# danieleschmidt/connectome-gnn-suite

Measured on AMD Instinct MI355X. Metric: training graphs/sec, 3-layer GCN, batch=4096x360-ROI connectomes, higher is better.
Workload: dtype f32; 1 GPU; cfg4-headline-gcn-4096x360-h64; model=gcn, rois=360, ws_k=14, edges_per_graph=5040, hidden=64, layers=3, node_order=dataset, graphs_per_gpu=4096, global_batch=4096, optimizer=Adam lr1e-3 wd1e-4 (optim.Adam), impl=fused, launch=eager, bn=per-rank, rccl_ranks=0, parallelism=graph-sharded dp1

## Files before the change

connectome_gnn_amd/csrc/common.h:

```cpp
#pragma once
#include <hip/hip_runtime.h>
#include <stdint.h>
#include "../../include/cgnn.h"

#define CGNN_WAVE 64

#define CGNN_CHECK_LAUNCH()                                   \
  do {                                                        \
    if (hipGetLastError() != hipSuccess) return CGNN_ELAUNCH; \
  } while (0)

#define CGNN_NEED_BYTES(ptr, have, need)                                   \
  do {                                                                     \
    if ((ptr) && (int64_t)(have) < (int64_t)(need)) return CGNN_EINVAL;    \
  } while (0)

static inline hipStream_t cgnn_stream(void* s) { return reinterpret_cast<hipStream_t>(s); }

#define CGNN_MAX_DEVICES 64
static inline int cgnn_device_ordinal() {
  int d = 0;
  if (hipGetDevice(&d) != hipSuccess || d < 0 || d >= CGNN_MAX_DEVICES) return 0;
  return d;
}

static inline int64_t cgnn_align_up(int64_t x, int64_t a) { return (x + a - 1) / a * a; }

__device__ __forceinline__ int cgnn_uniform(int v) { return __builtin_amdgcn_readfirstlane(v); }

__device__ __forceinline__ float cgnn_wave_sum(float v) {
#pragma unroll
  for (int o = 32; o > 0; o >>= 1) v += __shfl_xor(v, o, 64);
  return v;
}
__device__ __forceinline__ double cgnn_wave_sum(double v) {
#pragma unroll
  for (int o = 32; o > 0; o >>= 1) v += __shfl_xor(v, o, 64);
  return v;
}

__device__ __forceinline__ double block_sum256(double v, double* sh) {
  v = cgnn_wave_sum(v);
  if ((threadIdx.x & 63) == 0) sh[threadIdx.x >> 6] = v;
  __syncthreads();
  const double t = sh[0] + sh[1] + sh[2] + sh[3];
  __syncthreads();
  return t;
}

typedef float cgnn_f32x4 __attribute__((ext_vector_type(4)));
typedef uint32_t cgnn_u32x4 __attribute__((ext_vector_type(4)));
typedef uint32_t cgnn_u32x2 __attribute__((ext_vector_type(2)));
__device__ __forceinline__ float4 ldnt4(const float* p) {
  const cgnn_f32x4 v = __builtin_nontemporal_load(reinterpret_cast<const cgnn_f32x4*>(p));
  return make_float4(v[0], v[1], v[2], v[3]);
}
__device__ __forceinline__ void stnt4(float* p, const float4& v) {
  __builtin_nontemporal_store(cgnn_f32x4{v.x, v.y, v.z, v.w}, reinterpret_cast<cgnn_f32x4*>(p));
}
__device__ __forceinline__ float ldnt(const float* p) { return __builtin_nontemporal_load(p); }
__device__ __forceinline__ uint4 ldnt(const uint4* p) {
  const cgnn_u32x4 v = __builtin_nontemporal_load(reinterpret_cast<const cgnn_u32x4*>(p));
  return make_uint4(v[0], v[1], v[2], v[3]);
}
__device__ __forceinline__ uint2 ldnt(const uint2* p) {
  const cgnn_u32x2 v = __builtin_nontemporal_load(reinterpret_cast<const cgnn_u32x2*>(p));
  return make_uint2(v[0], v[1]);
}
```

connectome_gnn_amd/csrc/fused_gcn.hip:

```cpp
#include "common.h"
#include "agg_block.h"
#include "split_bf16.h"
#include "bn_coef.h"
#include "bn_tail.h"
#include "drop_ew.h"
#include "l0src.h"

#define PF_LD ld4
#define PF_ST st4
#define BW_LD ldnt4
#define BW_ST stnt4

#ifdef CGNN_STAMPS
__device__ unsigned long long g_stamps[1024 * 8 * 8];
#define CGNN_STAMP_DECL unsigned long long stamp_t_ = 0; (void)stamp_t_;
#define CGNN_STAMP_BEGIN() stamp_t_ = __builtin_amdgcn_s_memtime();
#define CGNN_STAMP(slot)                                                               \
  {                                                                                    \
    const unsigned long long now_ = __builtin_amdgcn_s_memtime();                      \
    if ((threadIdx.x & 63) == 0)                                                       \
      g_stamps[((size_t)blockIdx.x * 8 + (threadIdx.x >> 6)) * 8 + (slot)] += now_ - stamp_t_; \
    stamp_t_ = now_;                                                                   \
  }
#else
#define CGNN_STAMP_DECL
#define CGNN_STAMP_BEGIN()
#define CGNN_STAMP(slot)
#endif

namespace {

typedef float f32x4 __attribute__((ext_vector_type(4)));

constexpr int HID = CGNN_FUSED_HIDDEN;
constexpr int NWAVE = 8;
constexpr int NTHR = NWAVE * 64;
constexpr int SLD = 68;
constexpr int STG_FLOATS = 16 * SLD;

__device__ __forceinline__ float4 act4(const float4& y, const float4& a, const float4& b,
                                        uint32_t keep, float scale, float4& f) {
  float4 z, x;
  z.x = fmaf(a.x, y.x, b.x); z.y = fmaf(a.y, y.y, b.y);
  z.z = fmaf(a.z, y.z, b.z); z.w = fmaf(a.w, y.w, b.w);
  f.x = (z.x > 0.f && (keep & 1u)) ? scale : 0.f;
  f.y = (z.y > 0.f && (keep & 2u)) ? scale : 0.f;
  f.z = (z.z > 0.f && (keep & 4u)) ? scale : 0.f;
  f.w = (z.w > 0.f && (keep & 8u)) ? scale : 0.f;
  x.x = z.x * f.x; x.y = z.y * f.y; x.z = z.z * f.z; x.w = z.w * f.w;
  return x;
}

// ... 18 lines not shown
  __syncthreads();
  if (threadIdx.x < 128) {
    double t = 0.0;
#pragma unroll
    for (int w = 0; w < NW; ++w) t += red[w * 128 + threadIdx.x];
    slab_row[threadIdx.x] = t;
  }
  __syncthreads();
}

#define CGNN_FWD_G 4
#define CGNN_BWD_G 2
constexpr int FWD_G = CGNN_FWD_G;
constexpr int BWD_G = CGNN_BWD_G;

template <int MAXR, bool FIRST>
__global__ void __launch_bounds__(NTHR) k_gcn_fwd(
    cgnn_tiles t, const float* __restrict__ Xin, int F0, const float* __restrict__ bn_prev,
    DropCfg drop_in, int use_drop, uint8_t* __restrict__ mask_out, const float* __restrict__ W,
    const float* __restrict__ bias, float* __restrict__ Y, double* __restrict__ stat_slab) {
  const DropCfg drop = drop_resolve(drop_in);
  __shared__ __attribute__((aligned(16))) float tile[MAXR * HID];
  __shared__ __attribute__((aligned(16))) float stg_all[NWAVE * STG_FLOATS];
  __shared__ float disl[MAXR];
  const int lane = threadIdx.x & 63, wave = threadIdx.x >> 6, q = lane >> 4, j = lane & 15;
  float* stg = stg_all + wave * STG_FLOATS;
  const uint4* ent = static_cast<const uint4*>(t.ent_dst);

  __shared__ __attribute__((aligned(16))) float Wt[FIRST ? 4 : HID * HID];
  float wreg[4][4];
  if (FIRST) {
#pragma unroll
    for (int tj = 0; tj < 4; ++tj)
#pragma unroll
      for (int s = 0; s < 4; ++s) {
        const int k = 4 * s + q;
        wreg[tj][s] = k < F0 ? W[(4 * j + tj) * F0 + k] : 0.f;
      }
  } else {
    for (int i = threadIdx.x; i < HID * HID; i += NTHR) Wt[(i & 63) * HID + (i >> 6)] = W[i];
  }
  const float4 bias4 = ld4(bias + 4 * j);
  float4 pa = make_float4(0.f, 0.f, 0.f, 0.f), pb = pa;
  if (!FIRST) {
    pa = ld4(bn_prev + 4 * j);
    pb = ld4(bn_prev + HID + 4 * j);
  }
  double s1[4] = {0, 0, 0, 0}, s2[4] = {0, 0, 0, 0};
  CGNN_STAMP_DECL
  constexpr int PF = FIRST ? 1 : MAXR / 32;
  float4 pfy[PF];
  float pfd[PF];
  if (!FIRST && (int)blockIdx.x < t.num_tiles) {
    const int nb2 = t.tile_ptr[blockIdx.x], nn2 = t.tile_ptr[blockIdx.x + 1] - nb2;
#pragma unroll
    for (int u = 0; u < PF; ++u) {
      const int row = (threadIdx.x >> 4) + 32 * u;
      pfy[u] = make_float4(0.f, 0.f, 0.f, 0.f);
      pfd[u] = 0.f;
      if (row < nn2) {
        pfy[u] = ld4(Xin + (int64_t)(nb2 + row) * HID + 4 * j);
        pfd[u] = t.dis[nb2 + row];
      }
    }
  }

  for (int tid = blockIdx.x; tid < t.num_tiles; tid += gridDim.x) {
    CGNN_STAMP_BEGIN()
    const int base = t.tile_ptr[tid];
    const int n = t.tile_ptr[tid + 1] - base;
    const int nblk = (n + 15) >> 4;
    const int gb0 = t.tile_blk[tid];
    int boff[3] = {0, 0, 0}, bwid[3] = {0, 0, 0};
#pragma unroll
    for (int k = 0; k < 3; ++k) {
      const int bb = cgnn_uniform(wave) + NWAVE * k;
      if (bb < nblk) {
        boff[k] = t.blk_off_dst[gb0 + bb];
        bwid[k] = (t.blk_off_dst[gb0 + bb + 1] - boff[k]) >> 4;
      }
    }
    int off0 = boff[0], width = bwid[0], bk = 0;
    MetaRegs pre;
    if (wave < nblk) pre = meta_issue<true>(ent + (off0 >> 1), width, q, j);

    if (FIRST) {
      for (int r = threadIdx.x; r < nblk * 16; r += NTHR) disl[r] = r < n ? t.dis[base + r] : 0.f;
      for (int b = wave; b < nblk; b += NWAVE) {
        const int arow = 16 * b + j;
        f32x4 acc[4] = {{0, 0, 0, 0}, {0, 0, 0, 0}, {0, 0, 0, 0}, {0, 0, 0, 0}};
        float av[4], dv[4];
#pragma unroll
        for (int s = 0; s < 4; ++s) {
          const int k = 4 * s + q;
          av[s] = (arow < n && k < F0) ? Xin[(int64_t)(base + arow) * F0 + k] : 0.f;
          const int row = 16 * b + 4 * q + s;
          dv[s] = row < n ? t.dis[base + row] : 0.f;
        }
#pragma unroll
        for (int s = 0; s < 4; ++s)
          if (4 * s < F0) {
#pragma unroll
            for (int tj = 0; tj < 4; ++tj)
              acc[tj] = __builtin_amdgcn_mfma_f32_16x16x4f32(av[s], wreg[tj][s], acc[tj], 0, 0, 0);
          }
#pragma unroll
        for (int r = 0; r < 4; ++r)
          st4(tile + (16 * b + 4 * q + r) * HID + 4 * j,
              make_float4(acc[0][r] * dv[r], acc[1][r] * dv[r], acc[2][r] * dv[r], acc[3][r] * dv[r]));
      }
    } else {
#pragma unroll
      for (int u = 0; u < PF; ++u) {
        const int row = (threadIdx.x >> 4) + 32 * u;
        if (row < nblk * 16) {
          float4 x = make_float4(0.f, 0.f, 0.f, 0.f);
          if (row < n) {
            uint32_t keep = 0xFu;
            if (use_drop) {
              keep = drop_bits(drop, (uint32_t)(base + row) * 16u + (uint32_t)j);
              if (mask_out) mask_out[(int64_t)(base + row) * 16 + j] = (uint8_t)keep;
            }
            float4 f;
            x = scale4(act4(pfy[u], pa, pb, keep, drop.scale, f), pfd[u]);
          }
          st4(tile + row * HID + 4 * j, x);
          if (j == 0) disl[row] = pfd[u];
        }
      }
    }
    __syncthreads();
    if (!FIRST) {
      const int nxt = tid + gridDim.x;
      if (nxt < t.num_tiles) {
        const int nb2 = t.tile_ptr[nxt], nn2 = t.tile_ptr[nxt + 1] - nb2;
#pragma unroll
        for (int u = 0; u < PF; ++u) {
          const int row = (threadIdx.x >> 4) + 32 * u;
          pfy[u] = make_float4(0.f, 0.f, 0.f, 0.f);
          pfd[u] = 0.f;
          if (row < nn2) {
            pfy[u] = ld4(Xin + (int64_t)(nb2 + row) * HID + 4 * j);
            pfd[u] = t.dis[nb2 + row];
          }
        }
      }
    }
    CGNN_STAMP(1)

    for (int b = wave; b < nblk; b += NWAVE) {
      f32x4 acc[4] = {{0, 0, 0, 0}, {0, 0, 0, 0}, {0, 0, 0, 0}, {0, 0, 0, 0}};
      ++bk;
      const int off1 = bk == 1 ? boff[1] : boff[2], width1 = bk == 1 ? bwid[1] : bwid[2];
      CGNN_STAMP(2)
      float4 ag[4];
      agg_block<FWD_G, true>(tile, pre, ent + (off0 >> 1), width, q, j, ag);
      CGNN_STAMP(3)
      if (b + NWAVE < nblk) pre = meta_issue<true>(ent + (off1 >> 1), width1, q, j);
      off0 = off1; width = width1;
      if (FIRST) {
#pragma unroll
        for (int it = 0; it < 4; ++it) {
          const int row = 16 * b + 4 * q + it;
          if (row < n) {
            const float4 a = scale4(ag[it], disl[row]);
            const float4 y = make_float4(a.x + bias4.x, a.y + bias4.y, a.z + bias4.z, a.w + bias4.w);
            st4(Y + (int64_t)(base + row) * HID + 4 * j, y);
            s1[0] += y.x; s1[1] += y.y; s1[2] += y.z; s1[3] += y.w;
            s2[0] += (double)y.x * y.x; s2[1] += (double)y.y * y.y;
            s2[2] += (double)y.z * y.z; s2[3] += (double)y.w * y.w;
          }
        }
        CGNN_STAMP(4)
        continue;
      }
#pragma unroll
      for (int it = 0; it < 4; ++it)
        st4(stg + (4 * q + it) * SLD + 4 * j, scale4(ag[it], disl[16 * b + 4 * q + it]));
      __builtin_amdgcn_wave_barrier();
      float af[16];
#pragma unroll
      for (int u = 0; u < 4; ++u) {
        const float4 v = ld4(stg + j * SLD + 16 * q + 4 * u);
        af[4 * u + 0] = v.x; af[4 * u + 1] = v.y; af[4 * u + 2] = v.z; af[4 * u + 3] = v.w;
      }
      CGNN_STAMP(4)
#pragma unroll
      for (int s = 0; s < 16; ++s) {
// ... 45 lines not shown
}

constexpr int WSP_FRAGS = 3 * 2 * 4 * 64;
template <bool TRANSPOSED>
__device__ __forceinline__ void stage_split_weight(uint4* wsp, const float* __restrict__ W, int nthreads) {
  for (int idx = threadIdx.x; idx < 2 * 4 * 64; idx += nthreads) {
    const int ln = idx & 63, tj = (idx >> 6) & 3, ms = idx >> 8;
    const int qq = ln >> 4, jj = ln & 15;
    float v[8];
#pragma unroll
    for (int e = 0; e < 8; ++e) {
      const int k = 16 * (2 * ms + (e >> 2)) + 4 * qq + (e & 3), n = 4 * jj + tj;
      v[e] = TRANSPOSED ? W[k * HID + n] : W[n * HID + k];
    }
    const Split8 s = split8(make_float4(v[0], v[1], v[2], v[3]), make_float4(v[4], v[5], v[6], v[7]));
    wsp[((0 * 2 + ms) * 4 + tj) * 64 + ln] = s.h;
    wsp[((1 * 2 + ms) * 4 + tj) * 64 + ln] = s.m;
    wsp[((2 * 2 + ms) * 4 + tj) * 64 + ln] = s.l;
  }
}

constexpr int PF_NW = 12;
constexpr int PF_NTHR = PF_NW * 64;
#define CGNN_PF_G 2

template <int MAXR, bool FROM_P0>
__global__ void __launch_bounds__(PF_NTHR) k_gcn_fwd_pf(
    cgnn_tiles t, const float* __restrict__ Xin, cgnn_l0src l0, const float* __restrict__ bn_prev, DropCfg drop_in,
    int use_drop, uint8_t* __restrict__ mask_out, const float* __restrict__ W,
    const float* __restrict__ bias, float* __restrict__ Y, double* __restrict__ stat_slab, cgnn_bn_tail tail) {
  const DropCfg drop = drop_resolve(drop_in);
  __shared__ __attribute__((aligned(16))) float tile[MAXR * HID];
  __shared__ uint4 wsp[WSP_FRAGS];
  __shared__ __attribute__((aligned(16))) float bnab[2 * HID];
  __shared__ float disl[MAXR];
  const int lane = threadIdx.x & 63, wave = threadIdx.x >> 6, q = lane >> 4, j = lane & 15;
  const uint4* ent = static_cast<const uint4*>(t.ent_dst);
  constexpr int BPW = (MAXR / 16 + PF_NW - 1) / PF_NW;

  __shared__ __attribute__((aligned(16))) float b0l[FROM_P0 ? HID : 4];
  stage_split_weight<false>(wsp, W, PF_NTHR);
  for (int i = threadIdx.x; i < 2 * HID; i += PF_NTHR) bnab[i] = bn_prev[i];
  L0W w0;
  if (FROM_P0) {
    w0 = l0w_cols(l0, lane);
    for (int i = threadIdx.x; i < HID; i += PF_NTHR) b0l[i] = l0.b0[i];
  }
  const float4 bias4 = ld4(bias + 4 * j);
  double s1[4] = {0, 0, 0, 0}, s2[4] = {0, 0, 0, 0};

  constexpr int NPX = FROM_P0 ? 1 : 4;
  float4 px[BPW][NPX];
  float pd[BPW];
  auto request_block = [&](int tid, int u) {
    const int nb2 = t.tile_ptr[tid], nn2 = t.tile_ptr[tid + 1] - nb2;
    const int row = 16 * (wave + PF_NW * u) + j;
    pd[u] = 0.f;
#pragma unroll
    for (int c = 0; c < NPX; ++c) px[u][c] = make_float4(0.f, 0.f, 0.f, 0.f);
    if (row < nn2) {
      if (FROM_P0) {
        const float* src = l0.P0 + (int64_t)(nb2 + row) * L0_FP + q;
        px[u][0].x = src[0];
        px[u][0].y = src[4];
      } else {
        const float* src = Xin + (int64_t)(nb2 + row) * HID + 4 * q;
#pragma unroll
        for (int c = 0; c < NPX; ++c) px[u][c] = PF_LD(src + 16 * c);
      }
      pd[u] = t.dis[nb2 + row];
    }
  };
  auto request = [&](int tid) {
#pragma unroll
    for (int u = 0; u < BPW; ++u) request_block(tid, u);
  };
  if ((int)blockIdx.x < t.num_tiles) request(blockIdx.x);
  __syncthreads();

  for (int tid = blockIdx.x; tid < t.num_tiles; tid += gridDim.x) {
    const int base = t.tile_ptr[tid];
    const int n = t.tile_ptr[tid + 1] - base;
    const int nblk = (n + 15) >> 4;
    const int gb0 = t.tile_blk[tid];
    int boff[BPW], bwid[BPW];
#pragma unroll
    for (int k = 0; k < BPW; ++k) {
      boff[k] = bwid[k] = 0;
      const int bb = cgnn_uniform(wave) + PF_NW * k;
      if (bb < nblk) {
        boff[k] = t.blk_off_dst[gb0 + bb];
        bwid[k] = (t.blk_off_dst[gb0 + bb + 1] - boff[k]) >> 4;
      }
    }
    MetaRegs pre;
    if (wave < nblk) pre = meta_issue<true>(ent + (boff[0] >> 1), bwid[0], q, j);

    const int nxt = tid + gridDim.x;
#pragma unroll
    for (int u = 0; u < BPW; ++u) {
      const int b = wave + PF_NW * u;
      if (b >= nblk) break;
      const int row = 16 * b + j;
      const bool live = row < n;
      f32x4 acc[4] = {{0, 0, 0, 0}, {0, 0, 0, 0}, {0, 0, 0, 0}, {0, 0, 0, 0}};
#pragma unroll
      for (int ms = 0; ms < 2; ++ms) {
        float4 xc[2];
#pragma unroll
        for (int h2 = 0; h2 < 2; ++h2) {
          const int c = 2 * ms + h2;
          uint32_t keep = 0xFu;
          if (use_drop) {
            keep = drop_bits(drop, (uint32_t)(base + row) * 16u + (uint32_t)(4 * c + q));
            if (mask_out && live) mask_out[(int64_t)(base + row) * 16 + 4 * c + q] = (uint8_t)keep;
          }
          float4 f;
          float4 yraw = px[u][c < NPX ? c : 0];
          if (FROM_P0) {
            const float4 bq = ld4(b0l + 16 * c + 4 * q);
            const l0_f32x4 y0 = l0_mfma(w0.a[c], w0.b[c], px[u][0].x, px[u][0].y, l0_f32x4{bq.x, bq.y, bq.z, bq.w});
            yraw = make_float4(y0[0], y0[1], y0[2], y0[3]);
          }
          xc[h2] = scale4(act4(yraw, ld4(bnab + 16 * c + 4 * q), ld4(bnab + HID + 16 * c + 4 * q),
                               keep, drop.scale, f), pd[u]);
        }
        const Split8 a = split8(xc[0], xc[1]);
#pragma unroll
        for (int tj = 0; tj < 4; ++tj) {
          const uint4 bh = wsp[((0 * 2 + ms) * 4 + tj) * 64 + lane];
          const uint4 bm = wsp[((1 * 2 + ms) * 4 + tj) * 64 + lane];
          const uint4 bl = wsp[((2 * 2 + ms) * 4 + tj) * 64 + lane];
          acc[tj] = mfma_split(a, bh, bm, bl, acc[tj]);
        }
        __builtin_amdgcn_sched_barrier(0);
      }
#pragma unroll
      for (int r = 0; r < 4; ++r)
        st4(tile + (16 * b + 4 * q + r) * HID + 4 * j, make_float4(acc[0][r], acc[1][r], acc[2][r], acc[3][r]));
      if (q == 0) disl[row] = pd[u];
      if (nxt < t.num_tiles) request_block(nxt, u);
    }
    if (nxt < t.num_tiles) {
#pragma unroll
      for (int u = 0; u < BPW; ++u)
        if (wave + PF_NW * u >= nblk) request_block(nxt, u);
    }
    __syncthreads();

#pragma unroll
    for (int u = 0; u < BPW; ++u) {
      const int b = wave + PF_NW * u;
      if (b >= nblk) break;
      float4 ag[4];
      agg_block<CGNN_PF_G, true>(tile, pre, ent + (boff[u] >> 1), bwid[u], q, j, ag);
      if (u + 1 < BPW && b + PF_NW < nblk) pre = meta_issue<true>(ent + (boff[u + 1 < BPW ? u + 1 : u] >> 1), bwid[u + 1 < BPW ? u + 1 : u], q, j);
#pragma unroll
      for (int it = 0; it < 4; ++it) {
        const int row = 16 * b + 4 * q + it;
        if (row < n) {
          const float4 a = scale4(ag[it], disl[row]);
          const float4 y = make_float4(a.x + bias4.x, a.y + bias4.y, a.z + bias4.z, a.w + bias4.w);
          PF_ST(Y + (int64_t)(base + row) * HID + 4 * j, y);
          s1[0] += y.x; s1[1] += y.y; s1[2] += y.z; s1[3] += y.w;
          s2[0] += (double)y.x * y.x; s2[1] += (double)y.y * y.y;
          s2[2] += (double)y.z * y.z; s2[3] += (double)y.w * y.w;
        }
      }
    }
    __syncthreads();
  }
  if (tail.acc) {
    double* red = reinterpret_cast<double*>(tile);
    reduce_stats<double, PF_NW>(s1, s2, red, red + PF_NW * 128);
    bn_tail_run(tail, red + PF_NW * 128, reinterpret_cast<int*>(red + PF_NW * 128 + 128), [](int) { return 0.f; });
  } else if (stat_slab) {
    reduce_stats<double, PF_NW>(s1, s2, reinterpret_cast<double*>(tile), stat_slab + (int64_t)blockIdx.x * 128);
  }
}

struct PoolIn {
  const float* dP;
  const int32_t* node_graph;
  const int32_t* gptr;
  const uint8_t* mask_cur;
};

#ifndef CGNN_BWD_UNR
#define CGNN_BWD_UNR 4
#endif
#ifndef CGNN_BWD_UNR_POOL
#define CGNN_BWD_UNR_POOL 4
#endif
#ifndef CGNN_BWD_RO_G
#define CGNN_BWD_RO_G 8
#endif
constexpr int RO_G = CGNN_BWD_RO_G;


template <int MAXR, bool FIRST, bool POOLIN, bool XP0 = false, int NW = NWAVE>
__global__ void __launch_bounds__(NW * 64) k_gcn_bwd(
    cgnn_tiles t, PoolIn pin, cgnn_l0src l0, const float* __restrict__ dZ, const float* __restrict__ Y,
    const float* __restrict__ bn, const float* __restrict__ bwc,
    const float* __restrict__ Xprev , int F0,
    const float* __restrict__ bn_prev, DropCfg drop, int use_drop,
    const uint8_t* __restrict__ mask_prev, const float* __restrict__ W,
    float* __restrict__ dZprev, double* __restrict__ s_slab, float* __restrict__ dW_slab,
    double* __restrict__ db_slab, cgnn_bn_tail tail) {
  __shared__ __attribute__((aligned(16))) float tile[MAXR * HID];
  __shared__ __attribute__((aligned(16))) float stg_all[NW * STG_FLOATS];
  __shared__ uint4 wsp[FIRST ? 1 : WSP_FRAGS];
  __shared__ float disl[MAXR];
  const int lane = threadIdx.x & 63, wave = threadIdx.x >> 6, q = lane >> 4, j = lane & 15;
  float* stg = stg_all + wave * STG_FLOATS;
  const uint4* ent = static_cast<const uint4*>(t.ent_src);

  if (!FIRST) stage_split_weight<true>(wsp, W, (NW * 64));
  __shared__ __attribute__((aligned(16))) float bnl[FIRST ? 4 : 4 * HID];
  if (!FIRST) {
    for (int i = threadIdx.x; i < 4 * HID; i += (NW * 64)) bnl[i] = bn_prev[i];
  }
  __shared__ __attribute__((aligned(16))) float rog[POOLIN && RO_G > 0 ? RO_G * HID : 4];
  __shared__ int rog_g[2];
  auto stage_readout = [&](int tt) {
    const int nb = t.tile_ptr[tt], nn = t.tile_ptr[tt + 1] - nb;
    const int g0 = nn > 0 ? pin.node_graph[nb] : 0;
    const int ng = nn > 0 ? pin.node_graph[nb + nn - 1] - g0 + 1 : 0;
    if (ng <= RO_G) {
      for (int i = lane; i < ng * 16; i += 64) {
        const int g = g0 + (i >> 4), c = i & 15;
        const float inv = 1.0f / ((float)(pin.gptr[g + 1] - pin.gptr[g]) + 1e-8f);
        st4(rog + (i >> 4) * HID + 4 * c, scale4(ld4(pin.dP + (int64_t)g * HID + 4 * c), inv));
      }
    }
    if (lane == 0) {
      rog_g[0] = g0;
      rog_g[1] = ng <= RO_G;
    }
  };
  if (POOLIN) {
    if (cgnn_uniform(wave) == NW - 1 && (int)blockIdx.x < t.num_tiles) stage_readout(blockIdx.x);
    __syncthreads();
  }
  L0W w0;
  float4 b0q = make_float4(0.f, 0.f, 0.f, 0.f);
  if (XP0) {
    w0 = l0w_quad(l0, threadIdx.x & 63);
    b0q = ld4(l0.b0 + 4 * (threadIdx.x & 15));
  }
  f32x4 dw[4][FIRST ? 1 : 4];
#pragma unroll
  for (int a = 0; a < 4; ++a)
#pragma unroll
    for (int b2 = 0; b2 < (FIRST ? 1 : 4); ++b2) dw[a][b2] = f32x4{0, 0, 0, 0};
  float db[4] = {0, 0, 0, 0};
  float s1[4] = {0, 0, 0, 0}, s2[4] = {0, 0, 0, 0};
  CGNN_STAMP_DECL

  for (int tid = blockIdx.x; tid < t.num_tiles; tid += gridDim.x) {
    CGNN_STAMP_BEGIN()
    const int base = t.tile_ptr[tid];
    const int n = t.tile_ptr[tid + 1] - base;
    const int nblk = (n + 15) >> 4;
    const int gb0 = t.tile_blk[tid];
    const int uw = cgnn_uniform(wave);
    int off0 = 0, width = 0;
    if (uw < nblk) {
      off0 = t.blk_off_src[gb0 + uw];
      width = (t.blk_off_src[gb0 + uw + 1] - off0) >> 4;
    }
    MetaRegs pre;
    if (wave < nblk) pre = meta_issue<FIRST>(ent + (off0 >> 1), width, q, j);
    const int nxt = tid + gridDim.x;

    {
      const float4 ca = ld4(bn + 4 * j), cmean = ld4(bn + 2 * HID + 4 * j), cis = ld4(bn + 3 * HID + 4 * j);
      const float4 c1 = ld4(bwc + 4 * j), c2 = ld4(bwc + HID + 4 * j);
      const float4 cb = POOLIN ? ld4(bn + HID + 4 * j) : make_float4(0.f, 0.f, 0.f, 0.f);
      const int rg0 = POOLIN ? rog_g[0] : 0;
      const bool rstaged = POOLIN && rog_g[1] != 0;
      constexpr int UNR = POOLIN ? CGNN_BWD_UNR_POOL : CGNN_BWD_UNR;
      for (int r0 = threadIdx.x >> 4; r0 < nblk * 16; r0 += (NW * 4) * UNR) {
        float4 zb[UNR], yb[UNR];
        float dv[UNR];
        int gid[UNR];
        uint32_t kb[UNR];
#pragma unroll
        for (int u = 0; u < UNR; ++u) {
          const int row = r0 + (NW * 4) * u;
          zb[u] = yb[u] = make_float4(0.f, 0.f, 0.f, 0.f);
          dv[u] = 0.f;
          gid[u] = 0;
          kb[u] = 0xFu;
          if (row < n) {
            if (POOLIN) {
              gid[u] = pin.node_graph[base + row];
              if (use_drop) kb[u] = pin.mask_cur[(int64_t)(base + row) * 16 + j];
            } else {
              zb[u] = BW_LD(dZ + (int64_t)(base + row) * HID + 4 * j);
            }
            yb[u] = BW_LD(Y + (int64_t)(base + row) * HID + 4 * j);
            dv[u] = t.dis[base + row];
          }
        }
        if (POOLIN && rstaged) {
#pragma unroll
          for (int u = 0; u < UNR; ++u) {
            const int row = r0 + (NW * 4) * u;
            if (row < n) zb[u] = ld4(rog + (gid[u] - rg0) * HID + 4 * j);
          }
        } else if (POOLIN) {
#pragma unroll
          for (int u = 0; u < UNR; ++u) {
            const int row = r0 + (NW * 4) * u;
            if (row < n) {
              const float inv = 1.0f / ((float)(pin.gptr[gid[u] + 1] - pin.gptr[gid[u]]) + 1e-8f);
              zb[u] = scale4(ld4(pin.dP + (int64_t)gid[u] * HID + 4 * j), inv);
            }
          }
        }
#pragma unroll
        for (int u = 0; u < UNR; ++u) {
          const int row = r0 + (NW * 4) * u;
          if (row < nblk * 16) {
            float4 dy = make_float4(0.f, 0.f, 0.f, 0.f);
            if (row < n) {
              float4 dz = zb[u];
              const float4 y = yb[u];
              if (POOLIN) {
                float4 f;
                act4(y, ca, cb, kb[u], drop.scale, f);
                dz = make_float4(dz.x * f.x, dz.y * f.y, dz.z * f.z, dz.w * f.w);
              }
              dy.x = ca.x * (dz.x - c1.x - (y.x - cmean.x) * cis.x * c2.x);
              dy.y = ca.y * (dz.y - c1.y - (y.y - cmean.y) * cis.y * c2.y);
              dy.z = ca.z * (dz.z - c1.z - (y.z - cmean.z) * cis.z * c2.z);
              dy.w = ca.w * (dz.w - c1.w - (y.w - cmean.w) * cis.w * c2.w);
              db[0] += dy.x; db[1] += dy.y; db[2] += dy.z; db[3] += dy.w;
              dy = scale4(dy, dv[u]);
            }
            st4(tile + row * HID + 4 * j, dy);
            if (j == 0) disl[row] = dv[u];
          }
        }
      }
    }
    CGNN_STAMP(0)
    __syncthreads();
    CGNN_STAMP(1)

    for (int b = wave; b < nblk; b += NW) {
      float4 yp[4];
      float p0a = 0.f, p0b = 0.f;
      uint32_t keeps = 0u;
      {
        int off1 = 0, width1 = 0;
        {
          const int bn2 = cgnn_uniform(b) + NW;
          if (bn2 < nblk) {
            off1 = t.blk_off_src[gb0 + bn2];
            width1 = (t.blk_off_src[gb0 + bn2 + 1] - off1) >> 4;
          }
        }
        CGNN_STAMP(2)
        uint32_t kword = 0u;
        if (!FIRST) {
          if (16 * b + 4 * q + (j >> 2) < n) {
            kword = 0x0F0F0F0Fu;
            if (use_drop)
              kword = *reinterpret_cast<const uint32_t*>(mask_prev + (int64_t)(base + 16 * b + 4 * q) * 16 + 4 * j);
          }
#pragma unroll
          for (int r = 0; r < 4; ++r) {
            const int row = 16 * b + 4 * q + r;
            yp[r] = make_float4(0.f, 0.f, 0.f, 0.f);
            if (row < n && !XP0) yp[r] = BW_LD(Xprev + (int64_t)(base + row) * HID + 4 * j);
          }
        }
        if (!FIRST && XP0 && 16 * b + j < n) {
          const float* src = l0.P0 + (int64_t)(base + 16 * b + j) * L0_FP + q;
          p0a = src[0];
          p0b = src[4];
        }
        float4 ag[4];
        agg_block<FIRST ? 4 : BWD_G, FIRST>(tile, pre, ent + (off0 >> 1), width, q, j, ag);
        if (!FIRST) {
#pragma unroll
          for (int r = 0; r < 4; ++r) {
            const uint32_t v = (uint32_t)__shfl((int)kword, 16 * q + 4 * r + (j >> 2), 64);
            keeps |= ((v >> (8 * (j & 3))) & 0xFFu) << (8 * r);
          }
        }
        CGNN_STAMP(3)
        if (XP0) {
          l0_f32x4 yt[4];
#pragma unroll
          for (int tq = 0; tq < 4; ++tq) {
            const float bt = tq == 0 ? b0q.x : tq == 1 ? b0q.y : tq == 2 ? b0q.z : b0q.w;
            yt[tq] = l0_mfma(p0a, p0b, w0.a[tq], w0.b[tq], l0_f32x4{bt, bt, bt, bt});
          }
#pragma unroll
          for (int r = 0; r < 4; ++r) yp[r] = make_float4(yt[0][r], yt[1][r], yt[2][r], yt[3][r]);
        }
#pragma unroll
        for (int it = 0; it < 4; ++it)
          st4(stg + (4 * q + it) * SLD + 4 * j, scale4(ag[it], disl[16 * b + 4 * q + it]));
        if (b + NW < nblk) pre = meta_issue<FIRST>(ent + (off1 >> 1), width1, q, j);
        off0 = off1; width = width1;
      }
      __builtin_amdgcn_wave_barrier();

      if (FIRST) {
        float xv[4];
#pragma unroll
// ... 792 lines not shown
```

connectome_gnn_amd/csrc/fused_gcn_l0.hip:

```cpp
#include "common.h"
#include "l0src.h"
#include "bn_tail.h"

namespace {

constexpr int HID = CGNN_FUSED_HIDDEN;
constexpr int FP = 8;
constexpr int MAXR = CGNN_FUSED_MAX_ROWS;
constexpr int L0THR = 384;
constexpr int L0BTHR = 256;

__device__ __forceinline__ float4 ld4(const float* p) { return *reinterpret_cast<const float4*>(p); }
#define L0NT ldnt4
#define L0NTE(p) ldnt(p)
#define L0STNT stnt4
__device__ __forceinline__ void st4(float* p, const float4& v) { *reinterpret_cast<float4*>(p) = v; }

#define CGNN_L0_MINW 8
template <bool WRITE_Y>
__global__ void __launch_bounds__(L0THR, WRITE_Y ? 5 : CGNN_L0_MINW) k_l0_fwd(cgnn_tiles t, const float* __restrict__ X0, int F0,
                                                  const float* __restrict__ W0,
                                                  const float* __restrict__ bias,
                                                  float* __restrict__ P0, float* __restrict__ Y,
                                                  double* __restrict__ stat_slab,
                                                  const float* __restrict__ center,
                                                  float* __restrict__ w_eff,
                                                  float* __restrict__ mean_offset, cgnn_bn_tail tail) {
  __shared__ __attribute__((aligned(16))) float smem[2 * MAXR * FP];
  float* xs = smem;
  float* ps = smem + MAXR * FP;
  double* red = reinterpret_cast<double*>(smem);
  const int j = threadIdx.x & 15, rr = threadIdx.x >> 4;
  const uint2* ent = static_cast<const uint2*>(t.ent_dst);
  __shared__ __attribute__((aligned(16))) float wl[WRITE_Y ? L0_LDS_FLOATS : 4];
  if (WRITE_Y) l0_stage(wl, cgnn_l0src{nullptr, W0, bias, F0}, L0THR);
  typedef float f32x4 __attribute__((ext_vector_type(4)));
  constexpr int NM = FP + 1, NWV = L0THR / 64;
  __shared__ double macc[WRITE_Y ? 1 : NWV * NM * NM];
  if (!WRITE_Y)
    for (int i = threadIdx.x; i < NWV * NM * NM; i += L0THR) macc[i] = 0.0;
  constexpr int RC = FP - 1;
  __shared__ float cvec[FP];
  if (!WRITE_Y) {
    if (threadIdx.x < FP)
      cvec[threadIdx.x] = (center && (threadIdx.x < F0 || threadIdx.x == RC)) ? center[threadIdx.x] : 0.f;
    if (w_eff && blockIdx.x == 0 && threadIdx.x < HID) {
      double last = 0.0;
      for (int k = 0; k < F0; ++k) {
        const float wv = W0[threadIdx.x * F0 + k];
        w_eff[threadIdx.x * (F0 + 1) + k] = wv;
        last += (double)wv * (double)center[k];
      }
      w_eff[threadIdx.x * (F0 + 1) + F0] = (float)last;
      if (mean_offset)
        mean_offset[threadIdx.x] = (float)((double)bias[threadIdx.x] + (double)(float)last * (double)center[RC]);
    }
    __syncthreads();
  }
  const bool centred = !WRITE_Y && center != nullptr;
  float s1[4] = {0, 0, 0, 0};
  double s2[4] = {0, 0, 0, 0};

  for (int tid = blockIdx.x; tid < t.num_tiles; tid += gridDim.x) {
    const int base = t.tile_ptr[tid];
    const int n = t.tile_ptr[tid + 1] - base;
    const int gb0 = t.tile_blk[tid];
    {
      constexpr int NI = MAXR * FP / L0THR;
      constexpr int NB = WRITE_Y ? NI : NI / 2;
#pragma unroll
      for (int u0 = 0; u0 < NI; u0 += NB) {
        float xv[NB], dvv[NB];
#pragma unroll
        for (int u = 0; u < NB; ++u) {
          const int idx = threadIdx.x + L0THR * (u0 + u), r = idx >> 3, k = idx & 7;
          xv[u] = dvv[u] = 0.f;
          if (r < n && (k < F0 || (centred && k == RC))) {
            xv[u] = k < F0 ? X0[(int64_t)(base + r) * F0 + k] - (WRITE_Y ? 0.f : cvec[k]) : 1.f;
            dvv[u] = t.dis[base + r];
          }
        }
#pragma unroll
        for (int u = 0; u < NB; ++u) xs[threadIdx.x + L0THR * (u0 + u)] = xv[u] * dvv[u];
      }
    }
    __syncthreads();
    for (int r = threadIdx.x; r < n; r += L0THR) {
      const int b = r >> 4, i = r & 15;
      const int off0 = t.blk_off_dst[gb0 + b];
      const int width = (t.blk_off_dst[gb0 + b + 1] - off0) >> 4;
      float4 a0 = make_float4(0.f, 0.f, 0.f, 0.f), a1 = a0;
      double ar = 0.0;
      const uint2* e = ent + off0 + i;
#define CGNN_L0_EB 2
      constexpr int EB = WRITE_Y ? 6 : CGNN_L0_EB;
      for (int s0 = 0; s0 < width; s0 += EB) {
        uint2 eb[EB];
#pragma unroll
        for (int u = 0; u < EB; ++u) eb[u] = s0 + u < width ? L0NTE(e + 16 * (s0 + u)) : make_uint2(0u, 0u);
#pragma unroll
        for (int u = 0; u < EB; ++u) {
          const float w = __uint_as_float(eb[u].y);
          const float* src = xs + (eb[u].x >> 8) * FP;
          const float4 v0 = ld4(src), v1 = ld4(src + 4);
          a0.x = fmaf(w, v0.x, a0.x); a0.y = fmaf(w, v0.y, a0.y); a0.z = fmaf(w, v0.z, a0.z); a0.w = fmaf(w, v0.w, a0.w);
          a1.x = fmaf(w, v1.x, a1.x); a1.y = fmaf(w, v1.y, a1.y); a1.z = fmaf(w, v1.z, a1.z);
          if (WRITE_Y) a1.w = fmaf(w, v1.w, a1.w);
          else ar = fma((double)w, (double)v1.w, ar);
        }
      }
      const float dv = t.dis[base + r];
      a0 = make_float4(a0.x * dv, a0.y * dv, a0.z * dv, a0.w * dv);
      a1 = make_float4(a1.x * dv, a1.y * dv, a1.z * dv, a1.w * dv);
      if (!WRITE_Y) {
        if (centred) {
          const float rc = (float)(ar * (double)dv - (double)cvec[RC]);
          a0.y = F0 == 1 ? rc : a0.y; a0.z = F0 == 2 ? rc : a0.z; a0.w = F0 == 3 ? rc : a0.w;
          a1.x = F0 == 4 ? rc : a1.x; a1.y = F0 == 5 ? rc : a1.y; a1.z = F0 == 6 ? rc : a1.z;
          a1.w = F0 == 7 ? rc : 0.f;
        } else {
          a1.w = (float)(ar * (double)dv);
        }
      }
      st4(ps + r * FP, a0); st4(ps + r * FP + 4, a1);
      L0STNT(P0 + (int64_t)(base + r) * FP, a0); L0STNT(P0 + (int64_t)(base + r) * FP + 4, a1);
    }
    __syncthreads();
    if (!WRITE_Y) {
      if (stat_slab || tail.acc) {
        const int lane = threadIdx.x & 63, wave = threadIdx.x >> 6, ci = lane & 15, kq = lane >> 4;
        f32x4 acc = {0.f, 0.f, 0.f, 0.f};
        for (int rb = wave; 16 * rb < n; rb += L0THR / 64) {
#pragma unroll
          for (int g = 0; g < 4; ++g) {
            const int row = 16 * rb + 4 * g + kq;
            float v = 0.f;
            if (row < n) v = ci < FP ? ps[row * FP + ci] : (ci == FP ? 1.f : 0.f);
            acc = __builtin_amdgcn_mfma_f32_16x16x4f32(v, v, acc, 0, 0, 0);
          }
        }
#pragma unroll
        for (int r = 0; r < 4; ++r) {
          const int m = 4 * kq + r;
// ... 166 lines not shown
            }
          }
          const bool b0 = j & 1, b1 = j & 2;
          float h[4], tt[2];
#pragma unroll
          for (int k = 0; k < 4; ++k) {
            const float send = b0 ? g[k] : g[4 + k];
            h[k] = (b0 ? g[4 + k] : g[k]) + L0_DPP(send, 0xB1);
          }
#pragma unroll
          for (int k = 0; k < 2; ++k) {
            const float send = b1 ? h[k] : h[2 + k];
            tt[k] = (b1 ? h[2 + k] : h[k]) + L0_DPP(send, 0x4E);
          }
          tt[0] += L0_DPP(tt[0], 0x128); tt[1] += L0_DPP(tt[1], 0x128);
          tt[0] += L0_DPP(tt[0], 0x124); tt[1] += L0_DPP(tt[1], 0x124);
          if (j < 4) *reinterpret_cast<float2*>(G0 + row * FP + 4 * (j & 1) + (j & 2)) = make_float2(tt[0], tt[1]);
        }
      }
    }
  }
#pragma unroll
  for (int c = 0; c < 4; ++c) {
    redb[rr * HID + 4 * j + c] = (double)db[c];
#pragma unroll
    for (int k = 0; k < FP; ++k) redw[(rr * HID + 4 * j + c) * FP + k] = dw[c][k];
  }
  __syncthreads();
  for (int e = threadIdx.x; e < HID * FP; e += L0BTHR) {
    double tot = 0.0, ext = 0.0, dbt = 0.0;
    const int col = e / FP, k = e % FP;
#pragma unroll
    for (int r2 = 0; r2 < 16; ++r2) {
      tot += (double)redw[r2 * HID * FP + e];
      ext += (double)redw[r2 * HID * FP + col * FP + FT];
      dbt += redb[r2 * HID + col];
    }
    if (center && k < FT) tot += (double)shs[k] * (ext + (double)shs[FP - 1] * dbt);
    dW_slab[(int64_t)blockIdx.x * HID * FP + e] = (float)tot;
  }
  if (threadIdx.x < HID) {
    double tot = 0.0;
#pragma unroll
    for (int r2 = 0; r2 < 16; ++r2) tot += redb[r2 * HID + threadIdx.x];
    db_slab[(int64_t)blockIdx.x * HID + threadIdx.x] = tot;
  }
}

__global__ void __launch_bounds__(L0THR, CGNN_L0_MINW) k_l0_dx(cgnn_tiles t, const float* __restrict__ G0, int F0,
                                                               float* __restrict__ dX0) {
  __shared__ __attribute__((aligned(16))) float gs[MAXR * FP];
  const uint2* ent = static_cast<const uint2*>(t.ent_src);
  for (int tid = blockIdx.x; tid < t.num_tiles; tid += gridDim.x) {
    const int base = t.tile_ptr[tid];
    const int n = t.tile_ptr[tid + 1] - base;
    const int gb0 = t.tile_blk[tid];
    {
      constexpr int NI = MAXR * FP / 4 / L0THR;
      float4 gv[NI];
      float dvv[NI];
#pragma unroll
      for (int u = 0; u < NI; ++u) {
        const int idx = threadIdx.x + L0THR * u, r = idx >> 1;
        gv[u] = make_float4(0.f, 0.f, 0.f, 0.f);
        dvv[u] = 0.f;
        if (r < n) {
          gv[u] = ld4(G0 + (int64_t)(base + r) * FP + 4 * (idx & 1));
          dvv[u] = t.dis[base + r];
        }
      }
#pragma unroll
      for (int u = 0; u < NI; ++u)
        st4(gs + 4 * (threadIdx.x + L0THR * u),
            make_float4(gv[u].x * dvv[u], gv[u].y * dvv[u], gv[u].z * dvv[u], gv[u].w * dvv[u]));
    }
    __syncthreads();
    for (int r = threadIdx.x; r < n; r += L0THR) {
      const int b = r >> 4, i = r & 15;
      const int off0 = t.blk_off_src[gb0 + b];
      const int width = (t.blk_off_src[gb0 + b + 1] - off0) >> 4;
      float4 a0 = make_float4(0.f, 0.f, 0.f, 0.f), a1 = a0;
      const uint2* e = ent + off0 + i;
      constexpr int EB = CGNN_L0_EB;
      for (int s0 = 0; s0 < width; s0 += EB) {
        uint2 eb[EB];
#pragma unroll
        for (int u = 0; u < EB; ++u) eb[u] = s0 + u < width ? L0NTE(e + 16 * (s0 + u)) : make_uint2(0u, 0u);
#pragma unroll
        for (int u = 0; u < EB; ++u) {
          const float w = __uint_as_float(eb[u].y);
          const float* src = gs + (eb[u].x >> 8) * FP;
          const float4 v0 = ld4(src), v1 = ld4(src + 4);
          a0.x = fmaf(w, v0.x, a0.x); a0.y = fmaf(w, v0.y, a0.y); a0.z = fmaf(w, v0.z, a0.z); a0.w = fmaf(w, v0.w, a0.w);
          a1.x = fmaf(w, v1.x, a1.x); a1.y = fmaf(w, v1.y, a1.y); a1.z = fmaf(w, v1.z, a1.z); a1.w = fmaf(w, v1.w, a1.w);
        }
      }
      const float dv = t.dis[base + r];
      const float av[FP] = {a0.x * dv, a0.y * dv, a0.z * dv, a0.w * dv, a1.x * dv, a1.y * dv, a1.z * dv, a1.w * dv};
      float* out = dX0 + (int64_t)(base + r) * F0;
#pragma unroll
      for (int k = 0; k < FP; ++k)
        if (k < F0) out[k] = av[k];
    }
    __syncthreads();
  }
}

__global__ void __launch_bounds__(L0THR) k_l0_center(cgnn_tiles t, const float* __restrict__ X0, int F0,
                                                     float* __restrict__ center) {
  __shared__ float ds[MAXR];
  __shared__ double part[L0THR / 64][FP];
  const uint2* ent = static_cast<const uint2*>(t.ent_dst);
  int tid = 0;
  while (tid < t.num_tiles && t.tile_ptr[tid + 1] == t.tile_ptr[tid]) ++tid;
  if (tid >= t.num_tiles) {
    if (threadIdx.x < FP) center[threadIdx.x] = threadIdx.x == FP - 1 ? 1.f : 0.f;
    return;
  }
  const int base = t.tile_ptr[tid], n = t.tile_ptr[tid + 1] - base, gb0 = t.tile_blk[tid];
  for (int r = threadIdx.x; r < MAXR; r += L0THR) ds[r] = r < n ? t.dis[base + r] : 0.f;
  __syncthreads();
  double a[FP];
#pragma unroll
  for (int k = 0; k < FP; ++k) a[k] = 0.0;
  for (int r = threadIdx.x; r < n; r += L0THR) {
#pragma unroll
    for (int k = 0; k < FP - 1; ++k)
      if (k < F0) a[k] += (double)X0[(int64_t)(base + r) * F0 + k];
    const int b = r >> 4, i = r & 15;
    const int off0 = t.blk_off_dst[gb0 + b];
    const int width = (t.blk_off_dst[gb0 + b + 1] - off0) >> 4;
    double acc = 0.0;
    for (int s0 = 0; s0 < width; ++s0) {
// ... 117 lines not shown
```

Baseline: 2.373 million graphs/s.

## Use scalar constant loads for tile metadata and prefetch next-tile block offsets

Tile and block offset tables are now read through a constant-address-space helper, so uniform indices can compile to scalar loads instead of per-lane vector loads. In the aggregation prefetch kernel, the next tile's base, end and block offsets are loaded during the current tile, which moves metadata latency off the critical path. Row handling is specialized at compile time for blocks whose 16 rows are all live, skipping the per-row bounds checks there. The cost is more live registers and more complex control flow. The constant-space cast also assumes the metadata is read-only for the whole kernel.

```diff
diff --git a/connectome_gnn_amd/csrc/common.h b/connectome_gnn_amd/csrc/common.h
--- a/connectome_gnn_amd/csrc/common.h
+++ b/connectome_gnn_amd/csrc/common.h
@@ -27,6 +27,10 @@
 static inline int64_t cgnn_align_up(int64_t x, int64_t a) { return (x + a - 1) / a * a; }
 
 __device__ __forceinline__ int cgnn_uniform(int v) { return __builtin_amdgcn_readfirstlane(v); }
+
+__device__ __forceinline__ int cgnn_sload(const int32_t* p, int i) {
+  return ((const __attribute__((address_space(4))) int32_t*)p)[i];
+}
 
 __device__ __forceinline__ float cgnn_wave_sum(float v) {
 #pragma unroll
diff --git a/connectome_gnn_amd/csrc/fused_gcn.hip b/connectome_gnn_amd/csrc/fused_gcn.hip
--- a/connectome_gnn_amd/csrc/fused_gcn.hip
+++ b/connectome_gnn_amd/csrc/fused_gcn.hip
@@ -1,3 +1,4 @@
+#include <type_traits>
 #include "common.h"
 #include "agg_block.h"
 #include "split_bf16.h"
@@ -122,7 +123,7 @@
   float4 pfy[PF];
   float pfd[PF];
   if (!FIRST && (int)blockIdx.x < t.num_tiles) {
-    const int nb2 = t.tile_ptr[blockIdx.x], nn2 = t.tile_ptr[blockIdx.x + 1] - nb2;
+    const int nb2 = cgnn_sload(t.tile_ptr, blockIdx.x), nn2 = cgnn_sload(t.tile_ptr, blockIdx.x + 1) - nb2;
 #pragma unroll
     for (int u = 0; u < PF; ++u) {
       const int row = (threadIdx.x >> 4) + 32 * u;
@@ -137,17 +138,17 @@
 
   for (int tid = blockIdx.x; tid < t.num_tiles; tid += gridDim.x) {
     CGNN_STAMP_BEGIN()
-    const int base = t.tile_ptr[tid];
-    const int n = t.tile_ptr[tid + 1] - base;
+    const int base = cgnn_sload(t.tile_ptr, tid);
+    const int n = cgnn_sload(t.tile_ptr, tid + 1) - base;
     const int nblk = (n + 15) >> 4;
-    const int gb0 = t.tile_blk[tid];
+    const int gb0 = cgnn_sload(t.tile_blk, tid);
     int boff[3] = {0, 0, 0}, bwid[3] = {0, 0, 0};
 #pragma unroll
     for (int k = 0; k < 3; ++k) {
       const int bb = cgnn_uniform(wave) + NWAVE * k;
       if (bb < nblk) {
-        boff[k] = t.blk_off_dst[gb0 + bb];
-        bwid[k] = (t.blk_off_dst[gb0 + bb + 1] - boff[k]) >> 4;
+        boff[k] = cgnn_sload(t.blk_off_dst, gb0 + bb);
+        bwid[k] = (cgnn_sload(t.blk_off_dst, gb0 + bb + 1) - boff[k]) >> 4;
       }
     }
     int off0 = boff[0], width = bwid[0], bk = 0;
@@ -203,7 +204,7 @@
     if (!FIRST) {
       const int nxt = tid + gridDim.x;
       if (nxt < t.num_tiles) {
-        const int nb2 = t.tile_ptr[nxt], nn2 = t.tile_ptr[nxt + 1] - nb2;
+        const int nb2 = cgnn_sload(t.tile_ptr, nxt), nn2 = cgnn_sload(t.tile_ptr, nxt + 1) - nb2;
 #pragma unroll
         for (int u = 0; u < PF; ++u) {
           const int row = (threadIdx.x >> 4) + 32 * u;
@@ -355,13 +356,12 @@
   constexpr int NPX = FROM_P0 ? 1 : 4;
   float4 px[BPW][NPX];
   float pd[BPW];
-  auto request_block = [&](int tid, int u) {
-    const int nb2 = t.tile_ptr[tid], nn2 = t.tile_ptr[tid + 1] - nb2;
+  auto request_block = [&](int nb2, int end2, int u) {
     const int row = 16 * (wave + PF_NW * u) + j;
     pd[u] = 0.f;
 #pragma unroll
     for (int c = 0; c < NPX; ++c) px[u][c] = make_float4(0.f, 0.f, 0.f, 0.f);
-    if (row < nn2) {
+    if (nb2 + row < end2) {
       if (FROM_P0) {
         const float* src = l0.P0 + (int64_t)(nb2 + row) * L0_FP + q;
         px[u][0].x = src[0];
@@ -374,36 +374,52 @@
       pd[u] = t.dis[nb2 + row];
     }
   };
-  auto request = [&](int tid) {
-#pragma unroll
-    for (int u = 0; u < BPW; ++u) request_block(tid, u);
+  const int uw = cgnn_uniform(wave);
+  int base = 0, end = 0;
+  int blo[BPW] = {}, bhi[BPW] = {};
+  auto block_offsets = [&](int g0, int nb, int (&lo)[BPW], int (&hi)[BPW]) {
+#pragma unroll
+    for (int k = 0; k < BPW; ++k) {
+      const int bb = uw + PF_NW * k;
+      const bool have = bb < nb;
+      const int g = have ? g0 + bb : 0;
+      lo[k] = cgnn_sload(t.blk_off_dst, g);
+      hi[k] = cgnn_sload(t.blk_off_dst, g + (have ? 1 : 0));
+    }
   };
-  if ((int)blockIdx.x < t.num_tiles) request(blockIdx.x);
+  if ((int)blockIdx.x < t.num_tiles) {
+    base = cgnn_sload(t.tile_ptr, blockIdx.x);
+    end = cgnn_sload(t.tile_ptr, blockIdx.x + 1);
+#pragma unroll
+    for (int u = 0; u < BPW; ++u) request_block(base, end, u);
+    block_offsets(cgnn_sload(t.tile_blk, blockIdx.x), (end - base + 15) >> 4, blo, bhi);
+  }
   __syncthreads();
+  asm volatile("" ::"v"(pd[BPW - 1]));
 
   for (int tid = blockIdx.x; tid < t.num_tiles; tid += gridDim.x) {
-    const int base = t.tile_ptr[tid];
-    const int n = t.tile_ptr[tid + 1] - base;
+    const int n = end - base;
     const int nblk = (n + 15) >> 4;
-    const int gb0 = t.tile_blk[tid];
     int boff[BPW], bwid[BPW];
 #pragma unroll
     for (int k = 0; k < BPW; ++k) {
-      boff[k] = bwid[k] = 0;
-      const int bb = cgnn_uniform(wave) + PF_NW * k;
-      if (bb < nblk) {
-        boff[k] = t.blk_off_dst[gb0 + bb];
-        bwid[k] = (t.blk_off_dst[gb0 + bb + 1] - boff[k]) >> 4;
-      }
-    }
-    MetaRegs pre;
-    if (wave < nblk) pre = meta_issue<true>(ent + (boff[0] >> 1), bwid[0], q, j);
-
+      boff[k] = blo[k];
+      bwid[k] = (bhi[k] - blo[k]) >> 4;
+    }
     const int nxt = tid + gridDim.x;
+    const bool has_next = nxt < t.num_tiles;
+    const int nx = has_next ? nxt : tid;
+    const int base2 = cgnn_sload(t.tile_ptr, nx), end2 = cgnn_sload(t.tile_ptr, nx + 1);
+    const int gb2 = cgnn_sload(t.tile_blk, nx);
+    const uint4 zero4 = make_uint4(0u, 0u, 0u, 0u);
+    MetaRegs pre{zero4, zero4, zero4, zero4};
+    const bool has_blk = uw < nblk;
+
 #pragma unroll
     for (int u = 0; u < BPW; ++u) {
-      const int b = wave + PF_NW * u;
-      if (b >= nblk) break;
+      const int b = uw + PF_NW * u;
+      if (u == 0 ? !has_blk : b >= nblk) break;
+      if (u == 0) pre = meta_issue<true>(ent + (boff[0] >> 1), bwid[0], q, j);
       const int row = 16 * b + j;
       const bool live = row < n;
       f32x4 acc[4] = {{0, 0, 0, 0}, {0, 0, 0, 0}, {0, 0, 0, 0}, {0, 0, 0, 0}};
@@ -442,36 +458,54 @@
       for (int r = 0; r < 4; ++r)
         st4(tile + (16 * b + 4 * q + r) * HID + 4 * j, make_float4(acc[0][r], acc[1][r], acc[2][r], acc[3][r]));
       if (q == 0) disl[row] = pd[u];
-      if (nxt < t.num_tiles) request_block(nxt, u);
-    }
-    if (nxt < t.num_tiles) {
+      if (u == 0) asm volatile("" ::"v"(pre.a1.w), "v"(pre.b1.w));
+      if (has_next) request_block(base2, end2, u);
+    }
+    if (has_next) {
 #pragma unroll
       for (int u = 0; u < BPW; ++u)
-        if (wave + PF_NW * u >= nblk) request_block(nxt, u);
+        if (uw + PF_NW * u >= nblk) request_block(base2, end2, u);
     }
     __syncthreads();
-
-#pragma unroll
-    for (int u = 0; u < BPW; ++u) {
-      const int b = wave + PF_NW * u;
-      if (b >= nblk) break;
-      float4 ag[4];
-      agg_block<CGNN_PF_G, true>(tile, pre, ent + (boff[u] >> 1), bwid[u], q, j, ag);
-      if (u + 1 < BPW && b + PF_NW < nblk) pre = meta_issue<true>(ent + (boff[u + 1 < BPW ? u + 1 : u] >> 1), bwid[u + 1 < BPW ? u + 1 : u], q, j);
-#pragma unroll
-      for (int it = 0; it < 4; ++it) {
-        const int row = 16 * b + 4 * q + it;
-        if (row < n) {
-          const float4 a = scale4(ag[it], disl[row]);
-          const float4 y = make_float4(a.x + bias4.x, a.y + bias4.y, a.z + bias4.z, a.w + bias4.w);
-          PF_ST(Y + (int64_t)(base + row) * HID + 4 * j, y);
-          s1[0] += y.x; s1[1] += y.y; s1[2] += y.z; s1[3] += y.w;
-          s2[0] += (double)y.x * y.x; s2[1] += (double)y.y * y.y;
-          s2[2] += (double)y.z * y.z; s2[3] += (double)y.w * y.w;
-        }
-      }
-    }
+    int blo2[BPW], bhi2[BPW];
+    block_offsets(gb2, has_next ? (end2 - base2 + 15) >> 4 : 0, blo2, bhi2);
+
+    auto block = [&](auto self, auto U) {
+      constexpr int u = decltype(U)::value;
+      if constexpr (u < BPW) {
+        const int b = uw + PF_NW * u;
+        float4 ag[4];
+        agg_block<CGNN_PF_G, true>(tile, pre, ent + (boff[u] >> 1), bwid[u], q, j, ag);
+        const bool all_rows = 16 * b + 16 <= n;
+        const bool more = u + 1 < BPW && all_rows && b + PF_NW < nblk;
+        if (more) pre = meta_issue<true>(ent + (boff[u + 1 < BPW ? u + 1 : u] >> 1), bwid[u + 1 < BPW ? u + 1 : u], q, j);
+        auto rows = [&](auto all_live) {
+#pragma unroll
+          for (int it = 0; it < 4; ++it) {
+            const int row = 16 * b + 4 * q + it;
+            if (decltype(all_live)::value || row < n) {
+              const float4 a = scale4(ag[it], disl[row]);
+              const float4 y = make_float4(a.x + bias4.x, a.y + bias4.y, a.z + bias4.z, a.w + bias4.w);
+              PF_ST(Y + (int64_t)(base + row) * HID + 4 * j, y);
+              s1[0] += y.x; s1[1] += y.y; s1[2] += y.z; s1[3] += y.w;
+              s2[0] += (double)y.x * y.x; s2[1] += (double)y.y * y.y;
+              s2[2] += (double)y.z * y.z; s2[3] += (double)y.w * y.w;
+            }
+          }
+        };
+        if (all_rows) {
+          rows(std::true_type{});
+          if (more) self(self, std::integral_constant<int, u + 1>{});
+        } else {
+          rows(std::false_type{});
+        }
+      }
+    };
+    if (has_blk) block(block, std::integral_constant<int, 0>{});
     __syncthreads();
+    base = base2; end = end2;
+#pragma unroll
+    for (int k = 0; k < BPW; ++k) { blo[k] = blo2[k]; bhi[k] = bhi2[k]; }
   }
   if (tail.acc) {
     double* red = reinterpret_cast<double*>(tile);
@@ -526,7 +560,7 @@
   __shared__ __attribute__((aligned(16))) float rog[POOLIN && RO_G > 0 ? RO_G * HID : 4];
   __shared__ int rog_g[2];
   auto stage_readout = [&](int tt) {
-    const int nb = t.tile_ptr[tt], nn = t.tile_ptr[tt + 1] - nb;
+    const int nb = cgnn_sload(t.tile_ptr, tt), nn = cgnn_sload(t.tile_ptr, tt + 1) - nb;
     const int g0 = nn > 0 ? pin.node_graph[nb] : 0;
     const int ng = nn > 0 ? pin.node_graph[nb + nn - 1] - g0 + 1 : 0;
     if (ng <= RO_G) {
@@ -562,15 +596,15 @@
 
   for (int tid = blockIdx.x; tid < t.num_tiles; tid += gridDim.x) {
     CGNN_STAMP_BEGIN()
-    const int base = t.tile_ptr[tid];
-    const int n = t.tile_ptr[tid + 1] - base;
+    const int base = cgnn_sload(t.tile_ptr, tid);
+    const int n = cgnn_sload(t.tile_ptr, tid + 1) - base;
     const int nblk = (n + 15) >> 4;
-    const int gb0 = t.tile_blk[tid];
+    const int gb0 = cgnn_sload(t.tile_blk, tid);
     const int uw = cgnn_uniform(wave);
     int off0 = 0, width = 0;
     if (uw < nblk) {
-      off0 = t.blk_off_src[gb0 + uw];
-      width = (t.blk_off_src[gb0 + uw + 1] - off0) >> 4;
+      off0 = cgnn_sload(t.blk_off_src, gb0 + uw);
+      width = (cgnn_sload(t.blk_off_src, gb0 + uw + 1) - off0) >> 4;
     }
     MetaRegs pre;
     if (wave < nblk) pre = meta_issue<FIRST>(ent + (off0 >> 1), width, q, j);
@@ -661,8 +695,8 @@
         {
           const int bn2 = cgnn_uniform(b) + NW;
           if (bn2 < nblk) {
-            off1 = t.blk_off_src[gb0 + bn2];
-            width1 = (t.blk_off_src[gb0 + bn2 + 1] - off1) >> 4;
+            off1 = cgnn_sload(t.blk_off_src, gb0 + bn2);
+            width1 = (cgnn_sload(t.blk_off_src, gb0 + bn2 + 1) - off1) >> 4;
           }
         }
         CGNN_STAMP(2)
diff --git a/connectome_gnn_amd/csrc/fused_gcn_l0.hip b/connectome_gnn_amd/csrc/fused_gcn_l0.hip
--- a/connectome_gnn_amd/csrc/fused_gcn_l0.hip
+++ b/connectome_gnn_amd/csrc/fused_gcn_l0.hip
@@ -62,9 +62,9 @@
   double s2[4] = {0, 0, 0, 0};
 
   for (int tid = blockIdx.x; tid < t.num_tiles; tid += gridDim.x) {
-    const int base = t.tile_ptr[tid];
-    const int n = t.tile_ptr[tid + 1] - base;
-    const int gb0 = t.tile_blk[tid];
+    const int base = cgnn_sload(t.tile_ptr, tid);
+    const int n = cgnn_sload(t.tile_ptr, tid + 1) - base;
+    const int gb0 = cgnn_sload(t.tile_blk, tid);
     {
       constexpr int NI = MAXR * FP / L0THR;
       constexpr int NB = WRITE_Y ? NI : NI / 2;
@@ -87,8 +87,8 @@
     __syncthreads();
     for (int r = threadIdx.x; r < n; r += L0THR) {
       const int b = r >> 4, i = r & 15;
-      const int off0 = t.blk_off_dst[gb0 + b];
-      const int width = (t.blk_off_dst[gb0 + b + 1] - off0) >> 4;
+      const int off0 = cgnn_sload(t.blk_off_dst, gb0 + b);
+      const int width = (cgnn_sload(t.blk_off_dst, gb0 + b + 1) - off0) >> 4;
       float4 a0 = make_float4(0.f, 0.f, 0.f, 0.f), a1 = a0;
       double ar = 0.0;
       const uint2* e = ent + off0 + i;
@@ -361,9 +361,9 @@
   __shared__ __attribute__((aligned(16))) float gs[MAXR * FP];
   const uint2* ent = static_cast<const uint2*>(t.ent_src);
   for (int tid = blockIdx.x; tid < t.num_tiles; tid += gridDim.x) {
-    const int base = t.tile_ptr[tid];
-    const int n = t.tile_ptr[tid + 1] - base;
-    const int gb0 = t.tile_blk[tid];
+    const int base = cgnn_sload(t.tile_ptr, tid);
+    const int n = cgnn_sload(t.tile_ptr, tid + 1) - base;
+    const int gb0 = cgnn_sload(t.tile_blk, tid);
     {
       constexpr int NI = MAXR * FP / 4 / L0THR;
       float4 gv[NI];
@@ -386,8 +386,8 @@
     __syncthreads();
     for (int r = threadIdx.x; r < n; r += L0THR) {
       const int b = r >> 4, i = r & 15;
-      const int off0 = t.blk_off_src[gb0 + b];
-      const int width = (t.blk_off_src[gb0 + b + 1] - off0) >> 4;
+      const int off0 = cgnn_sload(t.blk_off_src, gb0 + b);
+      const int width = (cgnn_sload(t.blk_off_src, gb0 + b + 1) - off0) >> 4;
       float4 a0 = make_float4(0.f, 0.f, 0.f, 0.f), a1 = a0;
       const uint2* e = ent + off0 + i;
       constexpr int EB = CGNN_L0_EB;
```

Measured after the change: 2.376 million graphs/s (median of 2 runs). Within noise of the previous version (+0.1%).
